# jiamiya/HOPE

Hardware: AMD Instinct MI355X
Metric: parallel env steps/sec (full CarParking step incl. obs + RS search) (higher is better)
Workload: dtype f64

## Files before the change

hope_amd/_lib.py:

```python
import ctypes as C
import os

from .build import lib_path

LIDAR_NUM, N_ACTION, N_ITER, UPSAMPLE, TARGET_DIM, RS_MAX_SEG = 120, 42, 10, 10, 5, 5
F_OBS_F64, F_ACTION_F64, F_PROFILE, F_IMAGE, F_OVERLAP = 0x1, 0x2, 0x4, 0x8, 0x10
STAGE_MOTION, STAGE_OBS, STAGE_REWARD, STAGE_RS, STAGE_ALL = 0x1, 0x2, 0x4, 0x8, 0xF
ACTION_PHYSICAL = 0x10
ACTION_RESCALE_F32 = 0x80
AUTO_REDRAW = 0x100
DEFER_RS = 0x200
STAGE_IMG = 0x40
STAGE_NO_CULL, STAGE_ONE_SCENE = 0x4000, 0x8000
IMG_SIZE, IMG_CHANNELS, TRAJ_RENDER_LEN = 64, 3, 20
AUTO_RESET = 0x20
KERNELS = ('k_kinematics', 'k_env_step', 'k_rs_words', 'k_rs_validate', 'k_bev_image', 'k_bev_prep', 'k_rs_compact', 'k_post', 'k_rs_segs', 'k_rs_screen')
ABI_VERSION = 8

EXPORTS = ['hope_env_create', 'hope_env_destroy', 'hope_last_error', 'hope_abi_version', 'hope_env_upload_tables',
           'hope_env_set_scenes', 'hope_env_step', 'hope_env_wait_rs', 'hope_env_last_step', 'hope_env_wait_rs_step', 'hope_env_download_n_obst', 'hope_env_queue_check', 'hope_env_reset_obs', 'hope_env_download_state',
           'hope_env_upload_state', 'hope_env_restart', 'hope_env_set_pool', 'hope_env_pool_staging', 'hope_env_commit_pool', 'hope_env_commit_pool_relaxed', 'hope_env_pool_staging_ready', 'hope_env_pool_generation', 'hope_env_redraw', 'hope_env_set_redraw_seed', 'hope_env_download_pool_index', 'hope_env_set_dlp_cases', 'hope_env_pool_overflow', 'hope_env_set_draw_class', 'hope_env_download_scenes', 'hope_env_download_pool_state', 'hope_env_restore_maps', 'hope_env_kernel_ms', 'hope_env_kernel_union_ms', 'hope_env_profile_kernels', 'hope_debug_math', 'hope_debug_geom', 'hope_debug_traffic', 'hope_debug_mask_lut', 'hope_debug_rs_prof', 'hope_debug_rs_log', 'hope_debug_rs_filter_stats', 'hope_debug_rs_filter_dump', 'hope_debug_step_prof', 'hope_debug_census', 'hope_scenegen_generate', 'hope_scenegen_default_threads', 'hope_scenegen_generate_det', 'hope_scenegen_generate_device', 'hope_scenegen_log_det', 'hope_env_generate_pool', 'hope_env_curriculum_enable', 'hope_env_curriculum_disable', 'hope_env_set_pool_buckets', 'hope_env_curriculum_tally', 'hope_env_curriculum_update', 'hope_env_curriculum_state', 'hope_env_curriculum_set_windows', 'hope_env_curriculum_download_lists', 'hope_curriculum_lists_host', 'hope_curriculum_fold_host', 'hope_map_level_host', 'hope_map_level_device', 'hope_env_map_level', 'hope_env_planner_enable', 'hope_env_planner_disable', 'hope_env_planner_reset', 'hope_env_planner_step', 'hope_planner_step_host', 'hope_env_planner_download_state', 'hope_env_chooser_enable', 'hope_env_chooser_disable', 'hope_env_choose', 'hope_chooser_host', 'hope_env_obsnorm_enable', 'hope_env_obsnorm_disable', 'hope_env_obsnorm_set', 'hope_env_obsnorm_get', 'hope_env_obsnorm', 'hope_obsnorm_host', 'hope_env_num_scenes', 'hope_env_max_obstacles', 'hope_env_device_arch']


CURRICULUM_LIST_LEN = 1 << 20
PLAN_STATE_WORDS, PLAN_STEP_RATIO, PLAN_FORCED, PLAN_NO_POP = 6, 1.25, 0x1, 0x2
CHOOSE_NOMASK, CHOOSE_FIXED, CHOOSE_FALLBACK = 64, 128, 10
OBSNORM_LIDAR, OBSNORM_TARGET, OBSNORM_COLS, OBSNORM_UPDATE, OBSNORM_NORMALIZE = 120, 5, 125, 0x1, 0x2
BUCKET_UNLABELLED = 255


class HopeError(RuntimeError):
    pass


class StepOut(C.Structure):
    _fields_ = [('lidar', C.c_void_p), ('action_mask', C.c_void_p), ('target', C.c_void_p), ('reward', C.c_void_p),
# ... 130 lines not shown
```

hope_amd/csrc/hope_env.hip:

```cpp
#include <hip/hip_runtime.h>
#include <math.h>
#include <stdio.h>
#include <stdlib.h>
#include <string.h>

#include <algorithm>
#include <chrono>
#include <string>
#include <vector>

#include "hope_dev.h"
#include "hope_env.h"
#include "hope_internal.h"
#include "hope_step_kernel.h"
#include "hope_obs_pair.h"
#include "hope_motion_pair.h"
#include "hope_scenegen_kernel.h"
#include "hope_curriculum_kernel.h"
#include "hope_maplevel_kernel.h"
#include "hope_planner_kernel.h"
#include "hope_chooser_kernel.h"
#include "hope_obsnorm_kernel.h"

using namespace hope;
// ... 860 lines not shown
    hipError_t e = hipDeviceSynchronize();
    if (e == hipSuccess) e = hipMemcpyFromSymbol(buf, HIP_SYMBOL(g_census), sizeof(buf));
    for (int i = 0; i < 16; i++) {
        const bool is_min = i == 1 || i == 3 || i == 7;
        out[i] = is_min ? ~0ull : 0;
        for (int sh = 0; sh < 64; sh++) out[i] = is_min ? std::min<uint64_t>(out[i], buf[sh * 16 + i]) : out[i] + buf[sh * 16 + i];
    }
    if (e == hipSuccess && reset) {
        for (int sh = 0; sh < 64; sh++) for (int i = 0; i < 16; i++) buf[sh * 16 + i] = (i == 1 || i == 3 || i == 7) ? 0x7ff0000000000000ull : 0;
        e = hipMemcpyToSymbol(HIP_SYMBOL(g_census), buf, sizeof(buf));
    }
    return e == hipSuccess ? HOPE_OK : fail(HOPE_EHIP, std::string("hope_debug_census: ") + hipGetErrorString(e));
}

int hope_debug_rs_prof(uint64_t* out, int reset) {
    hipError_t e = rs_prof_read((unsigned long long*)out, reset);
    return e == hipSuccess ? HOPE_OK : fail(HOPE_EHIP, std::string("hope_debug_rs_prof: ") + hipGetErrorString(e));
}

int hope_debug_rs_filter_stats(uint64_t* out, int reset) {
    if (!out) return fail(HOPE_EINVAL, "hope_debug_rs_filter_stats: null argument");
    hipError_t e = rs_fstat_read((unsigned long long*)out, reset);
    return e == hipSuccess ? HOPE_OK : fail(HOPE_EHIP, std::string("hope_debug_rs_filter_stats: ") + hipGetErrorString(e));
}

int hope_debug_rs_filter_dump(double* out) {
    if (!out) return fail(HOPE_EINVAL, "hope_debug_rs_filter_dump: null argument");
    hipError_t e = rs_fdump_read(out);
    return e == hipSuccess ? HOPE_OK : fail(HOPE_EHIP, std::string("hope_debug_rs_filter_dump: ") + hipGetErrorString(e));
}

int hope_debug_rs_log(int32_t* out, int cap, int32_t* n, int reset) {
// ... 1914 lines not shown
```

hope_amd/csrc/hope_internal.h:

```cpp
#pragma once
#include <hip/hip_runtime.h>
#include <stdint.h>
#include "hope_env.h"

namespace hope {

constexpr uint32_t STAGE_NO_BEAMS = 0x1000;
constexpr uint32_t STAGE_NO_MASK = 0x2000;
constexpr uint32_t STAGE_NO_CULL = 0x4000;
constexpr uint32_t STAGE_ONE_SCENE = 0x8000;

struct RsWord {
    double len[5];
    double Lm;
    int code;
    int n;
    double pad;
};
constexpr int RS_WORDS_PER_SCENE = 48;
constexpr int RS_LIST_MAX_SCENES = 1 << 24;
__host__ __device__ inline int rs_list_pack(int scene, int n_obst) { return (int)(((unsigned)scene << 8) | (unsigned)n_obst); }
__host__ __device__ inline int rs_list_scene(int entry) { return (int)((unsigned)entry >> 8); }
__host__ __device__ inline int rs_list_n_obst(int entry) { return (int)((unsigned)entry & 0xFFu); }
constexpr int RS_IN_WORDS = 14;
// ... 50 lines not shown
    uint8_t* dyn;
    int32_t* layer_valid;
    int32_t* legacy_list;
    int32_t* rebuild;
    int* scratch;
    const uint8_t* active;
    uint8_t* img;
    int debug;
};

struct LaunchTimer {
    virtual void begin(int kind, hipStream_t s) = 0;
    virtual void end(hipStream_t s) = 0;
};
hipError_t launch_rs_search(const RsParams& p, hipStream_t stream, LaunchTimer* timer);
hipError_t rs_prof_read(unsigned long long* out , int reset);
hipError_t rs_init_tables();
hipError_t rs_fstat_read(unsigned long long* out , int reset);
hipError_t rs_fdump_read(double* out );
hipError_t rs_log_read(int* out , int cap, int* n, int reset);
size_t rs_lds_bytes(int max_obst);
size_t rs_screen_lds_bytes(int max_obst);
size_t rs_rec_bytes_per_scene();
hipError_t launch_bev_image(const BevParams& p, hipStream_t stream, LaunchTimer* timer, hipStream_t side = nullptr, hipEvent_t ev_fork = nullptr,
                            hipEvent_t ev_join = nullptr);
size_t bev_lds_bytes(bool legacy);

}
```

hope_amd/csrc/hope_rs.hip:

```cpp
#include <stdlib.h>

#include "hope_dev.h"
#include "hope_internal.h"

namespace hope {

namespace {

constexpr double MAXC = RS_MAXC;
constexpr double RS_STEP = 0.1;
constexpr double MAX_LENGTH = 1000.0;
constexpr int NCAND = 46;

enum { TS = 0, TL = 1, TR = 2 };

__device__ __forceinline__ double py_mod(double v, double w) {
    double m = hm_fmod(v, w);
    if (m != 0) { if ((w < 0) != (m < 0)) m += w; } else m = copysign(0.0, w);
    return m;
}
__device__ __forceinline__ double rs_M(double theta) {
    double phi = py_mod(theta, 2.0 * PI);
    if (phi < -PI) phi += 2.0 * PI;
    if (phi > PI) phi -= 2.0 * PI;
// ... 175 lines not shown
    v = fmaxf(v, dpp_f<0x141>(v));
    v = fmaxf(v, dpp_f<0x140>(v));
    const int i = __float_as_int(v);
    return fmaxf(fmaxf(__int_as_float(__builtin_amdgcn_readlane(i, 0)), __int_as_float(__builtin_amdgcn_readlane(i, 16))),
                 fmaxf(__int_as_float(__builtin_amdgcn_readlane(i, 32)), __int_as_float(__builtin_amdgcn_readlane(i, 48))));
}

__device__ __forceinline__ double wave_min_d(double v) {
    v = fmin(v, __hiloint2double(__builtin_amdgcn_mov_dpp(__double2hiint(v), 0xB1, 0xf, 0xf, true), __builtin_amdgcn_mov_dpp(__double2loint(v), 0xB1, 0xf, 0xf, true)));
    v = fmin(v, __hiloint2double(__builtin_amdgcn_mov_dpp(__double2hiint(v), 0x4E, 0xf, 0xf, true), __builtin_amdgcn_mov_dpp(__double2loint(v), 0x4E, 0xf, 0xf, true)));
    v = fmin(v, __hiloint2double(__builtin_amdgcn_mov_dpp(__double2hiint(v), 0x141, 0xf, 0xf, true), __builtin_amdgcn_mov_dpp(__double2loint(v), 0x141, 0xf, 0xf, true)));
    v = fmin(v, __hiloint2double(__builtin_amdgcn_mov_dpp(__double2hiint(v), 0x140, 0xf, 0xf, true), __builtin_amdgcn_mov_dpp(__double2loint(v), 0x140, 0xf, 0xf, true)));
    return fmin(fmin(readlane_d(v, 0), readlane_d(v, 16)), fmin(readlane_d(v, 32), readlane_d(v, 48)));
}

__device__ unsigned long long g_rs_prof[64 * 16];
constexpr int RS_LOG_CAP = 1 << 21;
__device__ int g_rs_log_n;
__device__ int4 g_rs_log[RS_LOG_CAP];
#define RS_T0() unsigned long long t0_ = TIMING ? __builtin_readcyclecounter() : 0
#define RS_T(i) do { if (TIMING) { const unsigned long long t1_ = __builtin_readcyclecounter(); tsec[i] += t1_ - t0_; t0_ = t1_; } } while (0)

template <bool TIMING, bool FULL = false>
__device__ __forceinline__ bool pose_hits(bool active, double wx, double wy, double wyaw, const double* tile,
                                          const float4* obb, int* cand, int n_obst, double xmin, double xmax,
                                          double ymin, double ymax, int lane, unsigned long long* tsec) {
    RS_T0();
    bool bad = false;
    double vx[4], vy[4];
    double hminx = INFINITY, hmaxx = -INFINITY, hminy = INFINITY, hmaxy = -INFINITY;
    if (active) {
// ... 322 lines not shown
        }
        if (k == 0) {
            tb[RS_SEGW + 7] = cq0;
            tb[2 * RS_SEGW + 7] = -sq0;
        }
    }
}

constexpr int RSB_SEG = 0, RSB_SEGW = RS_SEGW, RSB_QPD = RS_SEG_TABLE, RSB_QCAP = 256, RSB_BAD = RSB_QPD + RSB_QCAP;
constexpr int RSB_WORDS = RSB_BAD + 8;

template <int OCC, bool TIMING>
__global__ __launch_bounds__(64, OCC) void k_rs_validate(RsParams p, int obs_f64) {
    extern __shared__ __attribute__((aligned(16))) double lds[];
    const int lane = threadIdx.x;
    unsigned long long tsec[16] = {};
    const unsigned long long tstart_ = TIMING ? __builtin_readcyclecounter() : 0;
    RS_T0();
    const int count = *p.rs_count;
    if ((int)blockIdx.x >= count) return;
    if (obs_f64 & 0x400) return;
    const int qidx = scene_of_block(blockIdx.x, count);
    const int slot = p.slot_base + p.slot_dir * qidx;
    double* tile = lds;
    float4* obb = (float4*)(lds + 8 * p.tile_cap);
    double* scr = lds + 10 * p.tile_cap;
    double* segp = scr + RSB_SEG;
    double* qpd = scr + RSB_QPD;
    int* cand = (int*)(scr + RSB_WORDS);
    unsigned char* qseg = (unsigned char*)(cand + ((p.tile_cap + 3) & ~3));

// ... 125 lines not shown
                double cd = 0;
                unsigned char cs = 0;
                if (lane < rem) { cd = qpd[n + lane]; cs = qseg[n + lane]; }
                wsync();
                if (lane < rem) { qpd[lane] = cd; qseg[lane] = cs; }
                nq = rem;
            }
            wsync();
        }
        if (!invalid) { found = idx - 1; break; }
    }
    if (TIMING) {
        tsec[6] = __builtin_readcyclecounter() - tstart_;
        tsec[8] = 1;
        if (lane == 0) {
            for (int i = 0; i < 16; i++) if (tsec[i]) atomicAdd(&g_rs_prof[(blockIdx.x & 63) * 16 + i], tsec[i]);
            const int li = atomicAdd(&g_rs_log_n, 1);
            if (li < RS_LOG_CAP) g_rs_log[li] = make_int4((int)tsec[6], (int)tsec[9] | (n_paths << 8) | ((p.tile_cap > 32) << 16), (int)tsec[11], found >= 0);
        }
    }
    if (found < 0) return;

    const double wlen = lane < 5 ? segp[RSB_SEGW * lane + 6] : 0.0;
    const int code = __double2loint(segp[7]), nseg = __double2hiint(segp[7]);
    if (lane < 5) {
        double lm = lane < nseg ? wlen / MAXC : 0.0;
        if (p.rs_lengths) {
            if (obs_f64 & 1) ((double*)p.rs_lengths)[5 * (size_t)scene + lane] = lm;
            else ((float*)p.rs_lengths)[5 * (size_t)scene + lane] = (float)lm;
        }
        p.rs_word[8 * (size_t)scene + lane] = lane < nseg ? (int8_t)type_of(code, lane) : (int8_t)HOPE_RS_NONE;
    }
    if (lane == 5) p.rs_word[8 * (size_t)scene + 5] = (int8_t)nseg;
    if (lane == 6) p.rs_word[8 * (size_t)scene + 6] = 1;
}


constexpr float FEPS = 1e-3f, FKAPPA = 2e-2f, FETA_HULL = 2e-3f;
constexpr float F_INV_MAXC = (float)(1.0 / MAXC);
constexpr float F_HL = (float)(0.5 * (CAR_XF - CAR_XR)), F_HW = (float)CAR_YH, F_MID = (float)(0.5 * (CAR_XF + CAR_XR));
constexpr int RS_TAB = 256;
constexpr int RSB_TABF = RSB_BAD + 8, RSB_WORDS_F = RSB_TABF + RS_TAB;
constexpr int RSF_OCC = 4;
__device__ double g_rs_steps[RS_TAB];
__device__ unsigned long long g_rs_fstat[16];
__device__ double g_rs_fdump[64 * 16];

template <bool FULL>
__device__ __noinline__ bool exact_pass(int idx, const double* segp, const double* qpd, const unsigned char* qseg, double c_q,
                                        double s_q, double q0x, double q0y, double q0w, const double* verts_g,
                                        const float4* obb_g, int* cand, int n_obst, double xmin, double xmax, double ymin,
                                        double ymax, int lane) {
    const bool active = idx >= 0;
    double px = 0, py = 0, pyaw = 0;
    if (active) {
        const double spd = qpd[idx];
        const double* sp_ = segp + RSB_SEGW * (int)qseg[idx];
        const int m = (int)sp_[5];
        interpolate(spd, m, sp_[0], sp_[1], sp_[2], sp_[3], -sp_[4], sp_[3], sp_[4], px, py, pyaw);
// ... 67 lines not shown
            }
        }
    }
    return bad;
}

__device__ __forceinline__ double uni_d(double v) {
    return __hiloint2double(__builtin_amdgcn_readfirstlane(__double2hiint(v)), __builtin_amdgcn_readfirstlane(__double2loint(v)));
}

__device__ __forceinline__ void lsync() {
    asm volatile("s_waitcnt lgkmcnt(0)" ::: "memory");
    __builtin_amdgcn_wave_barrier();
}

constexpr double SCREEN_EPS = 1e-7;
constexpr int SCREEN_SPAN = 128;

__device__ __forceinline__ bool screen_obstacle_hit(const float4 v01, const float4 v23, float cx, float cy, float hc, float hs,
                                                    int efl, bool hull_ok) {
    constexpr float FEPS_ = FEPS, FKAPPA_ = FKAPPA, HL = F_HL, HW = F_HW;
    float u[4], w[4];
    {
        const float dx0 = v01.x - cx, dy0 = v01.y - cy, dx1 = v01.z - cx, dy1 = v01.w - cy;
        const float dx2 = v23.x - cx, dy2 = v23.y - cy, dx3 = v23.z - cx, dy3 = v23.w - cy;
        u[0] = hc * dx0 + hs * dy0; w[0] = hc * dy0 - hs * dx0;
        u[1] = hc * dx1 + hs * dy1; w[1] = hc * dy1 - hs * dx1;
        u[2] = hc * dx2 + hs * dy2; w[2] = hc * dy2 - hs * dx2;
        u[3] = hc * dx3 + hs * dy3; w[3] = hc * dy3 - hs * dx3;
    }
// ... 14 lines not shown
        const float ew0 = fminf(w[k], w[k2]), ew1 = fmaxf(w[k], w[k2]);
        const float esep = fmaxf(fmaxf(eu0 - HL, -HL - eu1), fmaxf(ew0 - HW, -HW - ew1));
        const float n1 = fabsf(nu) + fabsf(nw), mg = FEPS_ * n1;
        const bool clear = dn > mg || esep > FEPS_ || fmaxf(g[k], g[k2]) < -FEPS_;
        const bool cross = dn < -mg && esep < -FEPS_ && fminf(fabsf(g[k]), fabsf(g[k2])) > FEPS_ && fmaxf(g[k], g[k2]) > FEPS_;
        const float A = fabsf(nu) * HL, B = fabsf(nw) * HW;
        const bool corners_ok = fminf(fabsf(dn), fabsf(dist - fabsf(A - B))) > mg;
        const bool cross_u = fabsf(dist - A) <= B + mg, cross_w = fabsf(dist - B) <= A + mg;
        const bool angle_ok = (!cross_u || fabsf(nw) >= FKAPPA_ * n1) && (!cross_w || fabsf(nu) >= FKAPPA_ * n1);
        hit = hit || (!clear && cross && corners_ok && angle_ok && hull_ok && ((efl >> k) & 1));
    }
    return hit;
}

template <bool TIMING>
__device__ __forceinline__ unsigned long long screen_words(int lane, int n_paths, int n_obst, const double* tables, double* qpd, int* pq, int* cand,
                                                           const float2* fv, const float4* fbox, const unsigned char* eflag, float fxmax,
                                                           float fymax, unsigned long long* tsec) {
    const float fxmin = 0.0f, fymin = 0.0f;
    const double step = RS_STEP * MAXC;
    unsigned long long condemned = 0;
    RS_T0();
    const double inv_step = 1.0 / step;
    for (int w0 = 0; w0 < n_paths; w0 += 4) {
        const int nw = min(4, n_paths - w0);
        if (w0 > 0)
            for (int t = lane; t < RS_SEG_TABLE * nw; t += WAVE) qpd[t] = tables[RS_SEG_TABLE * w0 + t];
        lsync();
        RS_T(14);
        const int G = nw == 1 ? 64 : (nw == 2 ? 32 : (nw == 3 ? 21 : 16));
        const int stride = SCREEN_SPAN / G;
        const int wl_ = nw == 1 ? 0 : (nw == 2 ? lane >> 5 : (nw == 3 ? (lane >= 42 ? 2 : (lane >= 21 ? 1 : 0)) : lane >> 4));
        const int kk = lane - wl_ * G;
        const double* T = qpd + RS_SEG_TABLE * wl_;
        const double w7s = T[7];
        const int codew = __double2loint(w7s), nsegw = __double2hiint(w7s);
        const double a = (double)((kk + 1) * stride) * step;
        double c = 0.0, u0 = step, r = 0.0, lprev = 0.0, pdv = 0.0;
        int si = -1;
#pragma unroll
        for (int i = 0; i < 5; i++) {
            if (i < nsegw) {
                const double l = T[RS_SEGW * i + 6], al = fabs(l);
                if (i >= 1) u0 = (lprev * l > 0) ? r : -r;
// ... 78 lines not shown
                    classify(WAVE);
                    if (dead == all_w) { npq = 0; break; }
                    const int rem = npq - WAVE;
                    int cv = 0;
                    if (lane < rem) cv = pq[WAVE + lane];
                    lsync();
                    if (lane < rem) pq[lane] = cv;
                    npq = rem;
                }
            }
            if (npq > 0 && dead != all_w) { lsync(); classify(npq); }
        }
        condemned |= (unsigned long long)dead << w0;
        lsync();
        RS_T(7);
    }
    return condemned;
}

template <bool TIMING, int OCC = 8>
__global__ __launch_bounds__(64, OCC) void k_rs_screen(RsParams p) {
    extern __shared__ __attribute__((aligned(16))) double lds[];
    const int lane = threadIdx.x;
    unsigned long long tsec[16] = {};
    const int b_ = (int)blockIdx.x;
    const int qidx = scene_of_block(b_, p.max_queue);
    const int entry = p.rs_list[qidx];
    const int count = *p.rs_count;
    if (qidx >= count) return;
    const int slot = p.slot_base + p.slot_dir * qidx;
    const int scene = rs_list_scene(entry), n_obst = rs_list_n_obst(entry);
    float2* fv = (float2*)lds;
    float4* fbox = (float4*)(lds + 4 * p.tile_cap);
    double* tabs = lds + 6 * p.tile_cap;
    int* pq = (int*)(tabs + 4 * RS_SEG_TABLE);
    int* cand = pq + 2 * WAVE;
    unsigned char* eflag = (unsigned char*)(cand + ((p.tile_cap + 3) & ~3));
    double* rec = p.rs_rec + (size_t)slot * RS_REC_DOUBLES;
    const double r0 = lane < RS_REC_HDR ? rec[lane] : 0.0;
    const double* tables = rec + RS_REC_SEGS;
    {
        typedef __attribute__((address_space(3))) void* lds_ptr;
        const double2* t2 = (const double2*)tables;
        __builtin_amdgcn_global_load_lds((const void*)(t2 + lane), (lds_ptr)tabs, 16, 0, 0);
        if (lane < 2 * RS_SEG_TABLE - WAVE) __builtin_amdgcn_global_load_lds((const void*)(t2 + WAVE + lane), (lds_ptr)(tabs + 2 * WAVE), 16, 0, 0);
        const float4* gfv = p.fverts + (size_t)scene * p.max_obst * 2;
        const float4* gfb = p.fbox + (size_t)scene * p.max_obst;
        const uint32_t* gfl = (const uint32_t*)(p.eflag + (size_t)scene * eflag_stride(p.max_obst));
        float4* lfv = (float4*)fv;
        for (int base = 0; base < 2 * n_obst; base += WAVE)
            if (base + lane < 2 * n_obst) __builtin_amdgcn_global_load_lds((const void*)(gfv + base + lane), (lds_ptr)(lfv + base), 16, 0, 0);
        for (int base = 0; base < n_obst; base += WAVE)
            if (base + lane < n_obst) __builtin_amdgcn_global_load_lds((const void*)(gfb + base + lane), (lds_ptr)(fbox + base), 16, 0, 0);
        for (int base = 0; 4 * base < n_obst; base += WAVE)
            if (4 * (base + lane) < n_obst) __builtin_amdgcn_global_load_lds((const void*)(gfl + base + lane), (lds_ptr)((uint32_t*)eflag + base), 4, 0, 0);
    }
    asm volatile("s_waitcnt vmcnt(0)" ::: "memory");
    const int n_paths = __builtin_amdgcn_readlane(__double2hiint(r0), 1);
    if (n_paths == 0) return;
    const float fxmax = (float)(readlane_d(r0, 6) - readlane_d(r0, 5)), fymax = (float)(readlane_d(r0, 8) - readlane_d(r0, 7));
    lsync();
    const unsigned long long condemned = screen_words<TIMING>(lane, n_paths, n_obst, tables, tabs, pq, cand, fv, fbox, eflag, fxmax, fymax, tsec);
    if (lane == 0) {
        ((unsigned long long*)rec)[9] = condemned;
        if (condemned != ((1ull << n_paths) - 1)) p.surv_list[atomicAdd(p.surv_count, 1)] = make_int2(qidx, entry);
    }
}

template <int OCC, bool TIMING, bool STATS, bool PRE = false>
__global__ __launch_bounds__(64, OCC) void k_rs_validate_f(RsParams p, int obs_f64) {
    extern __shared__ __attribute__((aligned(16))) double lds[];
    const int lane = threadIdx.x;
    if (!(obs_f64 & 0x10000)) __builtin_amdgcn_s_setprio(1);
    unsigned long long tsec[16] = {};
    const unsigned long long tstart_ = TIMING ? __builtin_readcyclecounter() : 0;
    RS_T0();
    const int b_ = (int)blockIdx.x;
    int qidx, entry;
    if (PRE) {
        const int2 sv = p.surv_list[b_];
        if (b_ >= *p.surv_count) return;
        qidx = sv.x; entry = sv.y;
    } else {
#ifdef HOPE_RS_3TRIPS
        const int count = *p.rs_count;
        if (b_ >= count) return;
        qidx = scene_of_block(b_, count);
        entry = p.rs_list[qidx];
#else
// ... 17 lines not shown
    double* tabl = scr + RSB_TABF;
    unsigned char* qseg = (unsigned char*)(cand + ((p.tile_cap + 3) & ~3));
    unsigned char* eflag = qseg + RSB_QCAP;

    const double* rec = p.rs_rec + (size_t)slot * RS_REC_DOUBLES;
    const double r0 = lane < RS_REC_HDR ? rec[lane] : 0.0;
    const double* tables = rec + RS_REC_SEGS;
#ifdef HOPE_RS_3TRIPS
    if (__builtin_amdgcn_readlane(__double2hiint(r0), 1) == 0) return;
#endif
#ifdef HOPE_RS_HDR
    const int scene = __builtin_amdgcn_readlane(__double2loint(r0), 0);
    const int n_obst = __builtin_amdgcn_readlane(__double2hiint(r0), 0);
    (void)entry;
#endif
    double tb = lane < RS_SEG_TABLE ? tables[lane] : 0.0;
    if (!PRE) {
        typedef __attribute__((address_space(3))) void* lds_ptr;
        const double2* t2 = (const double2*)tables;
        __builtin_amdgcn_global_load_lds((const void*)(t2 + lane), (lds_ptr)qpd, 16, 0, 0);
        if (lane < 2 * RS_SEG_TABLE - WAVE) __builtin_amdgcn_global_load_lds((const void*)(t2 + WAVE + lane), (lds_ptr)(qpd + 2 * WAVE), 16, 0, 0);
    }
    {
        typedef __attribute__((address_space(3))) void* lds_ptr;
        const float4* gfv = p.fverts + (size_t)scene * p.max_obst * 2;
        const float4* gfb = p.fbox + (size_t)scene * p.max_obst;
        const uint32_t* gfl = (const uint32_t*)(p.eflag + (size_t)scene * eflag_stride(p.max_obst));
        float4* lfv = (float4*)fv;
        for (int base = 0; base < 2 * n_obst; base += WAVE)
            if (base + lane < 2 * n_obst) __builtin_amdgcn_global_load_lds((const void*)(gfv + base + lane), (lds_ptr)(lfv + base), 16, 0, 0);
        for (int base = 0; base < n_obst; base += WAVE)
            if (base + lane < n_obst) __builtin_amdgcn_global_load_lds((const void*)(gfb + base + lane), (lds_ptr)(fbox + base), 16, 0, 0);
        for (int base = 0; 4 * base < n_obst; base += WAVE)
            if (4 * (base + lane) < n_obst) __builtin_amdgcn_global_load_lds((const void*)(gfl + base + lane), (lds_ptr)((uint32_t*)eflag + base), 4, 0, 0);
    }
    const int n_paths = __builtin_amdgcn_readlane(__double2hiint(r0), 1);
    if (n_paths == 0) {
        asm volatile("s_waitcnt vmcnt(0)" ::: "memory");
        return;
    }
    const double* verts_g = p.verts + (size_t)scene * p.max_obst * 8;
    const float fxmin = 0.0f, fxmax = (float)(readlane_d(r0, 6) - readlane_d(r0, 5)), fymin = 0.0f, fymax = (float)(readlane_d(r0, 8) - readlane_d(r0, 7));
    const double step = RS_STEP * MAXC;
    bool tile_pending = true;
    int found = -1;
    double* bad1 = scr + RSB_BAD;
    if (lane < 6) bad1[lane] = INFINITY;
    lsync();
    RS_T(0);
    const bool paranoid = (obs_f64 & 0x2000) != 0;
    unsigned long long st_pass = 0, st_hit = 0, st_exact = 0, st_unc = 0, st_bad_hit = 0, st_bad_clear = 0, st_samples = 0;
    unsigned long long st_why[5] = {};
    unsigned long long condemned = 0;
    if (PRE) condemned = (unsigned long long)__double_as_longlong(readlane_d(r0, 9));
    else if (!(obs_f64 & 0x20000)) {
        asm volatile("s_waitcnt vmcnt(0)" ::: "memory");
        tile_pending = false;
        condemned = screen_words<TIMING>(lane, n_paths, n_obst, tables, qpd, (int*)tabl ,
                                         cand, fv, fbox, eflag, fxmax, fymax, tsec);
        if (TIMING) t0_ = __builtin_readcyclecounter();
    }
    else {
        asm volatile("s_waitcnt vmcnt(0)" ::: "memory");
        tile_pending = false;
    }
    const bool verify_screen = STATS && paranoid;
    const bool all_condemned = condemned == ((1ull << n_paths) - 1);
    unsigned long long st_scr_words = __popcll(condemned), st_scr_dead = all_condemned ? 1 : 0, st_scr_bad = 0;
    if (!all_condemned || verify_screen) {
        const double T0 = g_rs_steps[lane], T1 = g_rs_steps[WAVE + lane], T2 = g_rs_steps[2 * WAVE + lane], T3 = g_rs_steps[3 * WAVE + lane];
        tabl[lane] = T0; tabl[WAVE + lane] = T1; tabl[2 * WAVE + lane] = T2; tabl[3 * WAVE + lane] = T3;
        lsync();
    }
    for (int idx = 1; idx <= n_paths; idx++) {
        if (all_condemned && !verify_screen) break;
        const double tcur = tb;
        if (idx < n_paths && lane < RS_SEG_TABLE) tb = tables[RS_SEG_TABLE * idx + lane];
        const double len0 = readlane_d(tcur, 6), w6 = readlane_d(tcur, 7);
        const int code = __double2loint(w6), nseg = __double2hiint(w6);
        const int cls1 = type_of(code, 0) * 2 + (len0 > 0.0 ? 1 : 0);
        if (fabs(len0) >= bad1[cls1]) continue;
        const bool screened = (condemned >> (idx - 1)) & 1;
        if (screened && !verify_screen) continue;
        bool invalid = false;
        if (lane < RS_SEG_TABLE) segp[lane] = tcur;
        if (TIMING) tsec[9] += 1;
        {
            double zero;
            asm volatile("v_mov_b64 %0, 0" : "=v"(zero));
            if (lane == 0) { qpd[0] = zero; qseg[0] = (unsigned char)__double2loint(zero); }
        }
        int nq = 1;
        lsync();
        RS_T(1);
        const int win = 128;
        int i = 0, t_off = 0;
        bool seg_open = false, finished = false;
        double pd = 0, ll = 0.0, lprev = 0.0, d = 0, l = 0;
        while (!invalid && (!finished || nq > 0)) {
            while (!finished && nq + WAVE + 1 <= win) {
                if (TIMING) tsec[10] += 1;
                if (!seg_open) {
                    l = uni_d(segp[RSB_SEGW * i + 6]);
                    d = uni_d(l > 0.0 ? step : -step);
                    pd = uni_d((i >= 1 && (lprev * l) > 0) ? -d - ll : d - ll);
                    lprev = l;
                    seg_open = true;
                }
                double mine, t = pd;
                int ncap;
                if (i == 0 && t_off + WAVE <= RS_TAB) {
                    const double v = tabl[t_off + lane];
                    mine = d > 0.0 ? v : -v;
                    ncap = WAVE;
                    t_off += WAVE;
                    if (t_off < RS_TAB) {
                        const double nx = tabl[t_off];
                        t = d > 0.0 ? nx : -nx;
                    } else t = readlane_d(mine, WAVE - 1) + d;
                } else {
                    mine = pd;
                    double last = pd;
                    ncap = 0;
                    for (int j0 = 0; j0 < WAVE; j0 += 8) {
                        if ((lane >> 3) == (j0 >> 3)) mine = t;
#pragma unroll
                        for (int jj = 0; jj < 7; jj++) t = t + d;
                        last = t;
                        t = t + d;
                        ncap = j0 + 8;
                        if (__any(fabs(last) > fabs(l))) break;
                    }
#pragma unroll
                    for (int k = 0; k < 7; k++)
                        if (k < (lane & 7)) mine = mine + d;
                }
                const bool in_seg = lane < ncap && fabs(mine) <= fabs(l);
                const unsigned long long valid = (ncap == WAVE) ? ~0ull : ((1ull << ncap) - 1);
                const unsigned long long fail = ~__ballot(in_seg) & valid;
                const int cnt = fail ? (__ffsll((long long)fail) - 1) : ncap;
                if (lane < cnt) { qpd[nq + lane] = mine; qseg[nq + lane] = (unsigned char)i; }
                nq += cnt;
                if (fail) {
                    pd = readlane_d(mine, cnt);
                    ll = uni_d(l - pd - d);
                    seg_open = false;
                    if (i == nseg - 1) {
                        if (lane == 0) { qpd[nq] = l; qseg[nq] = (unsigned char)i; }
                        nq += 1;
                        finished = true;
// ... 184 lines not shown
            }
            {
                const int rem = n_all - n;
                double cd = 0;
                unsigned char cs = 0;
                if (lane < rem) { cd = qpd[n + lane]; cs = qseg[n + lane]; }
                lsync();
                if (lane < rem) { qpd[lane] = cd; qseg[lane] = cs; }
                nq = rem;
            }
            lsync();
        }
        if (STATS && screened && !invalid) { st_scr_bad += 1; continue; }
        if (!invalid) { found = idx - 1; break; }
    }
    if (STATS && lane == 0) {
        atomicAdd(&g_rs_fstat[7], st_scr_bad); atomicAdd(&g_rs_fstat[13], st_scr_words); atomicAdd(&g_rs_fstat[14], st_scr_dead);
        for (int b = 0; b < 5; b++) atomicAdd(&g_rs_fstat[8 + b], st_why[b]);
        atomicAdd(&g_rs_fstat[0], st_pass); atomicAdd(&g_rs_fstat[1], st_hit); atomicAdd(&g_rs_fstat[2], st_exact);
        atomicAdd(&g_rs_fstat[3], st_unc); atomicAdd(&g_rs_fstat[4], st_bad_hit); atomicAdd(&g_rs_fstat[5], st_bad_clear);
        atomicAdd(&g_rs_fstat[6], st_samples);
    }
    if (TIMING) {
        tsec[6] = __builtin_readcyclecounter() - tstart_;
        tsec[8] = 1;
        if (lane == 0) {
            for (int i = 0; i < 16; i++) if (tsec[i]) atomicAdd(&g_rs_prof[(blockIdx.x & 63) * 16 + i], tsec[i]);
            const int li = atomicAdd(&g_rs_log_n, 1);
            if (li < RS_LOG_CAP) g_rs_log[li] = make_int4((int)tsec[6], (int)tsec[9] | (n_paths << 8) | ((p.tile_cap > 32) << 16), (int)tsec[11], found >= 0);
        }
    }
    if (found < 0) return;
    const double wlen = lane < 5 ? segp[RSB_SEGW * lane + 6] : 0.0;
    const int code = __double2loint(segp[7]), nseg = __double2hiint(segp[7]);
    if (lane < 5) {
        double lm = lane < nseg ? wlen / MAXC : 0.0;
        if (p.rs_lengths) {
            if (obs_f64 & 1) ((double*)p.rs_lengths)[5 * (size_t)scene + lane] = lm;
            else ((float*)p.rs_lengths)[5 * (size_t)scene + lane] = (float)lm;
        }
        p.rs_word[8 * (size_t)scene + lane] = lane < nseg ? (int8_t)type_of(code, lane) : (int8_t)HOPE_RS_NONE;
    }
    if (lane == 5) p.rs_word[8 * (size_t)scene + 5] = (int8_t)nseg;
    if (lane == 6) p.rs_word[8 * (size_t)scene + 6] = 1;
}

}

static size_t rs_lds_bytes_exact(int max_obst) {
    return (size_t)(10 * max_obst + RSB_WORDS) * 8 + (size_t)((max_obst + 3) & ~3) * 4 + RSB_QCAP;
}
static size_t rs_lds_bytes_filter(int max_obst) {
    return (size_t)(6 * max_obst + RSB_WORDS_F) * 8 + (size_t)((max_obst + 3) & ~3) * 4 + RSB_QCAP + (size_t)((max_obst + 3) & ~3);
}
size_t rs_lds_bytes(int max_obst) { return std::max(rs_lds_bytes_exact(max_obst), rs_lds_bytes_filter(max_obst)); }
size_t rs_screen_lds_bytes(int max_obst) {
    return (size_t)(6 * max_obst + 4 * RS_SEG_TABLE) * 8 + 2 * WAVE * 4 + (size_t)((max_obst + 3) & ~3) * 4 + (size_t)((max_obst + 3) & ~3);
}
size_t rs_rec_bytes_per_scene() { return sizeof(double) * RS_REC_DOUBLES; }

hipError_t rs_prof_read(unsigned long long* out, int reset) {
    hipError_t e = hipDeviceSynchronize();
    if (e != hipSuccess) return e;
    static unsigned long long buf[64 * 16];
    e = hipMemcpyFromSymbol(buf, HIP_SYMBOL(g_rs_prof), sizeof(buf));
    for (int i = 0; i < 16; i++) { out[i] = 0; for (int sh = 0; sh < 64; sh++) out[i] += buf[sh * 16 + i]; }
    if (e == hipSuccess && reset) {
        for (auto& v : buf) v = 0;
        e = hipMemcpyToSymbol(HIP_SYMBOL(g_rs_prof), buf, sizeof(buf));
    }
    return e;
}

hipError_t rs_fdump_read(double* out ) {
    hipError_t e = hipDeviceSynchronize();
    if (e != hipSuccess) return e;
    return hipMemcpyFromSymbol(out, HIP_SYMBOL(g_rs_fdump), sizeof(double) * 64 * 16);
}

hipError_t rs_log_read(int* out , int cap, int* n, int reset) {
    hipError_t e = hipDeviceSynchronize();
// ... 87 lines not shown
```

include/hope_env.h:

```cpp
#ifndef HOPE_ENV_H
#define HOPE_ENV_H

#include <stdint.h>

#ifdef __cplusplus
extern "C" {
#endif

#define HOPE_ABI_VERSION 8

#define HOPE_LIDAR_NUM 120
#define HOPE_N_ACTION 42
#define HOPE_N_ITER 10
#define HOPE_UPSAMPLE 10
#define HOPE_TARGET_DIM 5
#define HOPE_RS_MAX_SEG 5
#define HOPE_IMG_SIZE 64
#define HOPE_IMG_CHANNELS 3
#define HOPE_TRAJ_RENDER_LEN 20

#define HOPE_OK 0
#define HOPE_EINVAL (-1)
#define HOPE_ENODEV (-2)
#define HOPE_ENOMEM (-3)
// ... 111 lines not shown
int hope_env_profile_kernels(hope_env_t *h, uint32_t kernel_mask);

int hope_env_download_state(hope_env_t *h, double *pose , int32_t *t ,
                            double *accum );
int hope_env_upload_state(hope_env_t *h, const double *pose, const int32_t *t, const double *accum);

int hope_debug_math(int fn, int n, const double *a, const double *b, double *out, void *stream);

int hope_debug_geom(int fn, int n, int n_obst, const double *in, void *out, void *stream);

int hope_debug_mask_lut(const double *dist_star, const double *hull_base, uint16_t *lut_out, double *scale_out);

int hope_debug_traffic(int mode, size_t bytes, void *buf, void *stream);

int hope_debug_rs_prof(uint64_t *out , int reset);
int hope_debug_rs_filter_stats(uint64_t *out , int reset);
int hope_debug_rs_filter_dump(double *out );
int hope_debug_rs_log(int32_t *out , int cap, int32_t *n, int reset);
int hope_debug_step_prof(uint64_t *out , int reset);
int hope_debug_census(uint64_t *out , int reset);

int hope_scenegen_generate(int level, int bay_mode, int n, uint64_t seed, int64_t first_index, int max_obstacles, double *start,
                           double *dest, double *bbox, double *verts, int32_t *n_obst, int32_t *case_id, int n_threads);
int hope_scenegen_default_threads(void);

int hope_scenegen_generate_det(int level, int bay_mode, int n, uint64_t seed, int64_t first_index, int max_obstacles, double *start,
                               double *dest, double *bbox, double *verts, int32_t *n_obst, int32_t *case_id, int n_threads);
int hope_scenegen_generate_device(int device_id, int level, int bay_mode, int n, uint64_t seed, int64_t first_index, int max_obstacles,
                                  double *start, double *dest, double *bbox, double *verts, int32_t *n_obst, int32_t *case_id, void *stream);
int hope_scenegen_log_det(int n, const double *x, double *y);
// ... 88 lines not shown
```

Measured before the change: 151.5 million.

## Double-buffer RS screen tables via LDS DMA and walk only surviving words

The screen loop now prefetches the next group of four word tables into a second LDS buffer with global_load_lds_dwordx4 while the current group is screened, instead of copying them with plain loads after a sync. The validate walk iterates only over uncondemned words using a bitmask, prefetching the next surviving word's table and reusing the table still resident in LDS. The step-sample table is loaded lazily by async DMA only when a word is actually walked, so fully condemned scenes skip it. It also adds more profiling slots and a walk-profile debug export. In exchange the screen kernel uses more LDS, which may lower occupancy, and the inline asm adds synchronisation subtleties.

```diff
diff --git a/hope_amd/_lib.py b/hope_amd/_lib.py
--- a/hope_amd/_lib.py
+++ b/hope_amd/_lib.py
@@ -19,7 +19,7 @@
 
 EXPORTS = ['hope_env_create', 'hope_env_destroy', 'hope_last_error', 'hope_abi_version', 'hope_env_upload_tables',
            'hope_env_set_scenes', 'hope_env_step', 'hope_env_wait_rs', 'hope_env_last_step', 'hope_env_wait_rs_step', 'hope_env_download_n_obst', 'hope_env_queue_check', 'hope_env_reset_obs', 'hope_env_download_state',
-           'hope_env_upload_state', 'hope_env_restart', 'hope_env_set_pool', 'hope_env_pool_staging', 'hope_env_commit_pool', 'hope_env_commit_pool_relaxed', 'hope_env_pool_staging_ready', 'hope_env_pool_generation', 'hope_env_redraw', 'hope_env_set_redraw_seed', 'hope_env_download_pool_index', 'hope_env_set_dlp_cases', 'hope_env_pool_overflow', 'hope_env_set_draw_class', 'hope_env_download_scenes', 'hope_env_download_pool_state', 'hope_env_restore_maps', 'hope_env_kernel_ms', 'hope_env_kernel_union_ms', 'hope_env_profile_kernels', 'hope_debug_math', 'hope_debug_geom', 'hope_debug_traffic', 'hope_debug_mask_lut', 'hope_debug_rs_prof', 'hope_debug_rs_log', 'hope_debug_rs_filter_stats', 'hope_debug_rs_filter_dump', 'hope_debug_step_prof', 'hope_debug_census', 'hope_scenegen_generate', 'hope_scenegen_default_threads', 'hope_scenegen_generate_det', 'hope_scenegen_generate_device', 'hope_scenegen_log_det', 'hope_env_generate_pool', 'hope_env_curriculum_enable', 'hope_env_curriculum_disable', 'hope_env_set_pool_buckets', 'hope_env_curriculum_tally', 'hope_env_curriculum_update', 'hope_env_curriculum_state', 'hope_env_curriculum_set_windows', 'hope_env_curriculum_download_lists', 'hope_curriculum_lists_host', 'hope_curriculum_fold_host', 'hope_map_level_host', 'hope_map_level_device', 'hope_env_map_level', 'hope_env_planner_enable', 'hope_env_planner_disable', 'hope_env_planner_reset', 'hope_env_planner_step', 'hope_planner_step_host', 'hope_env_planner_download_state', 'hope_env_chooser_enable', 'hope_env_chooser_disable', 'hope_env_choose', 'hope_chooser_host', 'hope_env_obsnorm_enable', 'hope_env_obsnorm_disable', 'hope_env_obsnorm_set', 'hope_env_obsnorm_get', 'hope_env_obsnorm', 'hope_obsnorm_host', 'hope_env_num_scenes', 'hope_env_max_obstacles', 'hope_env_device_arch']
+           'hope_env_upload_state', 'hope_env_restart', 'hope_env_set_pool', 'hope_env_pool_staging', 'hope_env_commit_pool', 'hope_env_commit_pool_relaxed', 'hope_env_pool_staging_ready', 'hope_env_pool_generation', 'hope_env_redraw', 'hope_env_set_redraw_seed', 'hope_env_download_pool_index', 'hope_env_set_dlp_cases', 'hope_env_pool_overflow', 'hope_env_set_draw_class', 'hope_env_download_scenes', 'hope_env_download_pool_state', 'hope_env_restore_maps', 'hope_env_kernel_ms', 'hope_env_kernel_union_ms', 'hope_env_profile_kernels', 'hope_debug_math', 'hope_debug_geom', 'hope_debug_traffic', 'hope_debug_mask_lut', 'hope_debug_rs_prof', 'hope_debug_rs_walk_prof', 'hope_debug_rs_log', 'hope_debug_rs_filter_stats', 'hope_debug_rs_filter_dump', 'hope_debug_step_prof', 'hope_debug_census', 'hope_scenegen_generate', 'hope_scenegen_default_threads', 'hope_scenegen_generate_det', 'hope_scenegen_generate_device', 'hope_scenegen_log_det', 'hope_env_generate_pool', 'hope_env_curriculum_enable', 'hope_env_curriculum_disable', 'hope_env_set_pool_buckets', 'hope_env_curriculum_tally', 'hope_env_curriculum_update', 'hope_env_curriculum_state', 'hope_env_curriculum_set_windows', 'hope_env_curriculum_download_lists', 'hope_curriculum_lists_host', 'hope_curriculum_fold_host', 'hope_map_level_host', 'hope_map_level_device', 'hope_env_map_level', 'hope_env_planner_enable', 'hope_env_planner_disable', 'hope_env_planner_reset', 'hope_env_planner_step', 'hope_planner_step_host', 'hope_env_planner_download_state', 'hope_env_chooser_enable', 'hope_env_chooser_disable', 'hope_env_choose', 'hope_chooser_host', 'hope_env_obsnorm_enable', 'hope_env_obsnorm_disable', 'hope_env_obsnorm_set', 'hope_env_obsnorm_get', 'hope_env_obsnorm', 'hope_obsnorm_host', 'hope_env_num_scenes', 'hope_env_max_obstacles', 'hope_env_device_arch']
 
 
 CURRICULUM_LIST_LEN = 1 << 20
diff --git a/hope_amd/csrc/hope_env.hip b/hope_amd/csrc/hope_env.hip
--- a/hope_amd/csrc/hope_env.hip
+++ b/hope_amd/csrc/hope_env.hip
@@ -898,8 +898,13 @@
 }
 
 int hope_debug_rs_prof(uint64_t* out, int reset) {
-    hipError_t e = rs_prof_read((unsigned long long*)out, reset);
+    hipError_t e = rs_prof_read((unsigned long long*)out, 0, 16, reset);
     return e == hipSuccess ? HOPE_OK : fail(HOPE_EHIP, std::string("hope_debug_rs_prof: ") + hipGetErrorString(e));
+}
+
+int hope_debug_rs_walk_prof(uint64_t* out, int reset) {
+    hipError_t e = rs_prof_read((unsigned long long*)out, 16, 8, reset);
+    return e == hipSuccess ? HOPE_OK : fail(HOPE_EHIP, std::string("hope_debug_rs_walk_prof: ") + hipGetErrorString(e));
 }
 
 int hope_debug_rs_filter_stats(uint64_t* out, int reset) {
diff --git a/hope_amd/csrc/hope_internal.h b/hope_amd/csrc/hope_internal.h
--- a/hope_amd/csrc/hope_internal.h
+++ b/hope_amd/csrc/hope_internal.h
@@ -88,7 +88,7 @@
     virtual void end(hipStream_t s) = 0;
 };
 hipError_t launch_rs_search(const RsParams& p, hipStream_t stream, LaunchTimer* timer);
-hipError_t rs_prof_read(unsigned long long* out , int reset);
+hipError_t rs_prof_read(unsigned long long* out , int first, int count, int reset);
 hipError_t rs_init_tables();
 hipError_t rs_fstat_read(unsigned long long* out , int reset);
 hipError_t rs_fdump_read(double* out );
diff --git a/hope_amd/csrc/hope_rs.hip b/hope_amd/csrc/hope_rs.hip
--- a/hope_amd/csrc/hope_rs.hip
+++ b/hope_amd/csrc/hope_rs.hip
@@ -213,7 +213,8 @@
     return fmin(fmin(readlane_d(v, 0), readlane_d(v, 16)), fmin(readlane_d(v, 32), readlane_d(v, 48)));
 }
 
-__device__ unsigned long long g_rs_prof[64 * 16];
+constexpr int RS_PROF_SLOTS = 24;
+__device__ unsigned long long g_rs_prof[64 * RS_PROF_SLOTS];
 constexpr int RS_LOG_CAP = 1 << 21;
 __device__ int g_rs_log_n;
 __device__ int4 g_rs_log[RS_LOG_CAP];
@@ -566,7 +567,7 @@
 __global__ __launch_bounds__(64, OCC) void k_rs_validate(RsParams p, int obs_f64) {
     extern __shared__ __attribute__((aligned(16))) double lds[];
     const int lane = threadIdx.x;
-    unsigned long long tsec[16] = {};
+    unsigned long long tsec[RS_PROF_SLOTS] = {};
     const unsigned long long tstart_ = TIMING ? __builtin_readcyclecounter() : 0;
     RS_T0();
     const int count = *p.rs_count;
@@ -722,7 +723,7 @@
         tsec[6] = __builtin_readcyclecounter() - tstart_;
         tsec[8] = 1;
         if (lane == 0) {
-            for (int i = 0; i < 16; i++) if (tsec[i]) atomicAdd(&g_rs_prof[(blockIdx.x & 63) * 16 + i], tsec[i]);
+            for (int i = 0; i < RS_PROF_SLOTS; i++) if (tsec[i]) atomicAdd(&g_rs_prof[(blockIdx.x & 63) * RS_PROF_SLOTS + i], tsec[i]);
             const int li = atomicAdd(&g_rs_log_n, 1);
             if (li < RS_LOG_CAP) g_rs_log[li] = make_int4((int)tsec[6], (int)tsec[9] | (n_paths << 8) | ((p.tile_cap > 32) << 16), (int)tsec[11], found >= 0);
         }
@@ -749,8 +750,10 @@
 constexpr float F_HL = (float)(0.5 * (CAR_XF - CAR_XR)), F_HW = (float)CAR_YH, F_MID = (float)(0.5 * (CAR_XF + CAR_XR));
 constexpr int RS_TAB = 256;
 constexpr int RSB_TABF = RSB_BAD + 8, RSB_WORDS_F = RSB_TABF + RS_TAB;
+constexpr int RSB_TABS2 = RSB_QPD + 4 * RS_SEG_TABLE, RSB_PQ = RSB_TABS2 + 4 * RS_SEG_TABLE;
+static_assert(RSB_PQ + WAVE <= RSB_TABF + RS_TAB, "the screen's second table buffer and pair queue (128 ints) end inside the sample table's words");
 constexpr int RSF_OCC = 4;
-__device__ double g_rs_steps[RS_TAB];
+__device__ __attribute__((aligned(16))) double g_rs_steps[RS_TAB];
 __device__ unsigned long long g_rs_fstat[16];
 __device__ double g_rs_fdump[64 * 16];
 
@@ -848,6 +851,19 @@
     __builtin_amdgcn_wave_barrier();
 }
 
+#pragma clang diagnostic push
+#pragma clang diagnostic ignored "-Winline-asm"
+__device__ __forceinline__ void lds_dma16(const void* src, const void* dst, int lane) {
+    typedef __attribute__((address_space(3))) const void* lds_cptr;
+    const unsigned m = __builtin_amdgcn_readfirstlane((unsigned)(unsigned long)(lds_cptr)dst);
+    const unsigned long a = (unsigned long)src;
+    const unsigned long sa = ((unsigned long)(unsigned)__builtin_amdgcn_readfirstlane((int)(a >> 32)) << 32) | (unsigned)__builtin_amdgcn_readfirstlane((int)a);
+    unsigned off;
+    asm volatile("s_mov_b32 m0, %2\n\tv_lshlrev_b32 %0, 4, %1\n\tglobal_load_lds_dwordx4 %0, %3"
+                 : "=&v"(off) : "v"(lane), "s"(m), "s"(sa) : "memory", "m0");
+}
+#pragma clang diagnostic pop
+
 constexpr double SCREEN_EPS = 1e-7;
 constexpr int SCREEN_SPAN = 128;
 
@@ -892,9 +908,9 @@
 }
 
 template <bool TIMING>
-__device__ __forceinline__ unsigned long long screen_words(int lane, int n_paths, int n_obst, const double* tables, double* qpd, int* pq, int* cand,
-                                                           const float2* fv, const float4* fbox, const unsigned char* eflag, float fxmax,
-                                                           float fymax, unsigned long long* tsec) {
+__device__ __forceinline__ unsigned long long screen_words(int lane, int n_paths, int n_obst, const double* tables, double* qpd, double* qpd2,
+                                                           int* pq, int* cand, const float2* fv, const float4* fbox, const unsigned char* eflag,
+                                                           float fxmax, float fymax, unsigned long long* tsec, const double** resident) {
     const float fxmin = 0.0f, fymin = 0.0f;
     const double step = RS_STEP * MAXC;
     unsigned long long condemned = 0;
@@ -902,10 +918,16 @@
     const double inv_step = 1.0 / step;
     for (int w0 = 0; w0 < n_paths; w0 += 4) {
         const int nw = min(4, n_paths - w0);
-        if (w0 > 0)
-            for (int t = lane; t < RS_SEG_TABLE * nw; t += WAVE) qpd[t] = tables[RS_SEG_TABLE * w0 + t];
+        if (w0 > 0) asm volatile("s_waitcnt vmcnt(0)" ::: "memory");
         lsync();
+        if (TIMING && w0 > 0) { tsec[19] += __builtin_readcyclecounter() - t0_; tsec[22] += 1; }
         RS_T(14);
+        if (w0 + 4 < n_paths) {
+            const int n2 = (RS_SEG_TABLE / 2) * min(4, n_paths - w0 - 4);
+            const double2* t2 = (const double2*)(tables + RS_SEG_TABLE * (w0 + 4));
+            if (lane < n2) lds_dma16(t2, qpd2, lane);
+            if (WAVE + lane < n2) lds_dma16(t2 + WAVE, qpd2 + 2 * WAVE, lane);
+        }
         const int G = nw == 1 ? 64 : (nw == 2 ? 32 : (nw == 3 ? 21 : 16));
         const int stride = SCREEN_SPAN / G;
         const int wl_ = nw == 1 ? 0 : (nw == 2 ? lane >> 5 : (nw == 3 ? (lane >= 42 ? 2 : (lane >= 21 ? 1 : 0)) : lane >> 4));
@@ -1014,7 +1036,9 @@
         condemned |= (unsigned long long)dead << w0;
         lsync();
         RS_T(7);
-    }
+        if (w0 + 4 < n_paths) { double* sw = qpd; qpd = qpd2; qpd2 = sw; }
+    }
+    *resident = qpd;
     return condemned;
 }
 
@@ -1022,7 +1046,7 @@
 __global__ __launch_bounds__(64, OCC) void k_rs_screen(RsParams p) {
     extern __shared__ __attribute__((aligned(16))) double lds[];
     const int lane = threadIdx.x;
-    unsigned long long tsec[16] = {};
+    unsigned long long tsec[RS_PROF_SLOTS] = {};
     const int b_ = (int)blockIdx.x;
     const int qidx = scene_of_block(b_, p.max_queue);
     const int entry = p.rs_list[qidx];
@@ -1033,7 +1057,7 @@
     float2* fv = (float2*)lds;
     float4* fbox = (float4*)(lds + 4 * p.tile_cap);
     double* tabs = lds + 6 * p.tile_cap;
-    int* pq = (int*)(tabs + 4 * RS_SEG_TABLE);
+    int* pq = (int*)(tabs + 8 * RS_SEG_TABLE);
     int* cand = pq + 2 * WAVE;
     unsigned char* eflag = (unsigned char*)(cand + ((p.tile_cap + 3) & ~3));
     double* rec = p.rs_rec + (size_t)slot * RS_REC_DOUBLES;
@@ -1060,7 +1084,9 @@
     if (n_paths == 0) return;
     const float fxmax = (float)(readlane_d(r0, 6) - readlane_d(r0, 5)), fymax = (float)(readlane_d(r0, 8) - readlane_d(r0, 7));
     lsync();
-    const unsigned long long condemned = screen_words<TIMING>(lane, n_paths, n_obst, tables, tabs, pq, cand, fv, fbox, eflag, fxmax, fymax, tsec);
+    const double* resident;
+    const unsigned long long condemned = screen_words<TIMING>(lane, n_paths, n_obst, tables, tabs, tabs + 4 * RS_SEG_TABLE, pq, cand, fv, fbox, eflag,
+                                                              fxmax, fymax, tsec, &resident);
     if (lane == 0) {
         ((unsigned long long*)rec)[9] = condemned;
         if (condemned != ((1ull << n_paths) - 1)) p.surv_list[atomicAdd(p.surv_count, 1)] = make_int2(qidx, entry);
@@ -1072,7 +1098,7 @@
     extern __shared__ __attribute__((aligned(16))) double lds[];
     const int lane = threadIdx.x;
     if (!(obs_f64 & 0x10000)) __builtin_amdgcn_s_setprio(1);
-    unsigned long long tsec[16] = {};
+    unsigned long long tsec[RS_PROF_SLOTS] = {};
     const unsigned long long tstart_ = TIMING ? __builtin_readcyclecounter() : 0;
     RS_T0();
     const int b_ = (int)blockIdx.x;
@@ -1120,7 +1146,6 @@
     const int n_obst = __builtin_amdgcn_readlane(__double2hiint(r0), 0);
     (void)entry;
 #endif
-    double tb = lane < RS_SEG_TABLE ? tables[lane] : 0.0;
     if (!PRE) {
         typedef __attribute__((address_space(3))) void* lds_ptr;
         const double2* t2 = (const double2*)tables;
@@ -1151,19 +1176,18 @@
     bool tile_pending = true;
     int found = -1;
     double* bad1 = scr + RSB_BAD;
-    if (lane < 6) bad1[lane] = INFINITY;
-    lsync();
     RS_T(0);
     const bool paranoid = (obs_f64 & 0x2000) != 0;
     unsigned long long st_pass = 0, st_hit = 0, st_exact = 0, st_unc = 0, st_bad_hit = 0, st_bad_clear = 0, st_samples = 0;
     unsigned long long st_why[5] = {};
     unsigned long long condemned = 0;
+    const double* resident = qpd;
     if (PRE) condemned = (unsigned long long)__double_as_longlong(readlane_d(r0, 9));
     else if (!(obs_f64 & 0x20000)) {
         asm volatile("s_waitcnt vmcnt(0)" ::: "memory");
         tile_pending = false;
-        condemned = screen_words<TIMING>(lane, n_paths, n_obst, tables, qpd, (int*)tabl ,
-                                         cand, fv, fbox, eflag, fxmax, fymax, tsec);
+        condemned = screen_words<TIMING>(lane, n_paths, n_obst, tables, qpd, scr + RSB_TABS2, (int*)(scr + RSB_PQ) ,
+                                         cand, fv, fbox, eflag, fxmax, fymax, tsec, &resident);
         if (TIMING) t0_ = __builtin_readcyclecounter();
     }
     else {
@@ -1171,23 +1195,50 @@
         tile_pending = false;
     }
     const bool verify_screen = STATS && paranoid;
-    const bool all_condemned = condemned == ((1ull << n_paths) - 1);
+    const unsigned long long all_words = (1ull << n_paths) - 1;
+    const bool all_condemned = condemned == all_words;
     unsigned long long st_scr_words = __popcll(condemned), st_scr_dead = all_condemned ? 1 : 0, st_scr_bad = 0;
-    if (!all_condemned || verify_screen) {
-        const double T0 = g_rs_steps[lane], T1 = g_rs_steps[WAVE + lane], T2 = g_rs_steps[2 * WAVE + lane], T3 = g_rs_steps[3 * WAVE + lane];
-        tabl[lane] = T0; tabl[WAVE + lane] = T1; tabl[2 * WAVE + lane] = T2; tabl[3 * WAVE + lane] = T3;
-        lsync();
-    }
-    for (int idx = 1; idx <= n_paths; idx++) {
-        if (all_condemned && !verify_screen) break;
+    unsigned long long todo = verify_screen ? all_words : (all_words & ~condemned);
+    if (TIMING && todo) tsec[21] += 1;
+    bool tabl_pending = false;
+    double tb = 0.0;
+    if (todo) {
+        const int first = __ffsll((long long)todo) - 1;
+        const int lds_w0 = (PRE || (obs_f64 & 0x20000)) ? 0 : ((n_paths - 1) & ~3);
+        if (!PRE && first >= lds_w0 && first < lds_w0 + 4) {
+            if (lane < RS_SEG_TABLE) tb = resident[RS_SEG_TABLE * (first - lds_w0) + lane];
+        } else if (lane < RS_SEG_TABLE) tb = tables[RS_SEG_TABLE * first + lane];
+    }
+    if (lane < 6) bad1[lane] = INFINITY;
+    lsync();
+    bool walked = false, tabl_requested = false;
+    while (todo) {
+        const unsigned long long tw_ = TIMING ? __builtin_readcyclecounter() : 0;
+        const int idx = __ffsll((long long)todo);
+        todo &= todo - 1;
+        if (tabl_pending && walked) {
+            asm volatile("s_waitcnt vmcnt(0)" ::: "memory");
+            tabl_pending = false;
+        }
         const double tcur = tb;
-        if (idx < n_paths && lane < RS_SEG_TABLE) tb = tables[RS_SEG_TABLE * idx + lane];
+        if (todo && lane < RS_SEG_TABLE) tb = tables[RS_SEG_TABLE * (__ffsll((long long)todo) - 1) + lane];
         const double len0 = readlane_d(tcur, 6), w6 = readlane_d(tcur, 7);
         const int code = __double2loint(w6), nseg = __double2hiint(w6);
+        if (TIMING) asm volatile("" :: "s"(code));
         const int cls1 = type_of(code, 0) * 2 + (len0 > 0.0 ? 1 : 0);
-        if (fabs(len0) >= bad1[cls1]) continue;
+        if (fabs(len0) >= bad1[cls1]) {
+            if (TIMING) { tsec[16] += __builtin_readcyclecounter() - tw_; tsec[20] += 1; }
+            continue;
+        }
         const bool screened = (condemned >> (idx - 1)) & 1;
-        if (screened && !verify_screen) continue;
+        if (!tabl_requested) {
+            const double2* g2 = (const double2*)g_rs_steps;
+            lds_dma16(g2, tabl, lane);
+            lds_dma16(g2 + WAVE, tabl + 2 * WAVE, lane);
+            tabl_requested = tabl_pending = true;
+        }
+        if (TIMING) tsec[18] += __builtin_readcyclecounter() - tw_;
+        walked = true;
         bool invalid = false;
         if (lane < RS_SEG_TABLE) segp[lane] = tcur;
         if (TIMING) tsec[9] += 1;
@@ -1215,7 +1266,17 @@
                 }
                 double mine, t = pd;
                 int ncap;
+#ifdef HOPE_RS_TABLE_WAIT
                 if (i == 0 && t_off + WAVE <= RS_TAB) {
+#else
+                if (i == 0 && t_off + WAVE <= RS_TAB && !(tabl_pending && t_off == 0)) {
+#endif
+                    if (tabl_pending) {
+                        const unsigned long long ts_ = TIMING ? __builtin_readcyclecounter() : 0;
+                        asm volatile("s_waitcnt vmcnt(0)" ::: "memory");
+                        tabl_pending = false;
+                        if (TIMING) tsec[17] += __builtin_readcyclecounter() - ts_;
+                    }
                     const double v = tabl[t_off + lane];
                     mine = d > 0.0 ? v : -v;
                     ncap = WAVE;
@@ -1240,6 +1301,7 @@
 #pragma unroll
                     for (int k = 0; k < 7; k++)
                         if (k < (lane & 7)) mine = mine + d;
+                    if (i == 0) t_off += WAVE;
                 }
                 const bool in_seg = lane < ncap && fabs(mine) <= fabs(l);
                 const unsigned long long valid = (ncap == WAVE) ? ~0ull : ((1ull << ncap) - 1);
@@ -1454,6 +1516,7 @@
         if (STATS && screened && !invalid) { st_scr_bad += 1; continue; }
         if (!invalid) { found = idx - 1; break; }
     }
+    if (tabl_pending) asm volatile("s_waitcnt vmcnt(0)" ::: "memory");
     if (STATS && lane == 0) {
         atomicAdd(&g_rs_fstat[7], st_scr_bad); atomicAdd(&g_rs_fstat[13], st_scr_words); atomicAdd(&g_rs_fstat[14], st_scr_dead);
         for (int b = 0; b < 5; b++) atomicAdd(&g_rs_fstat[8 + b], st_why[b]);
@@ -1465,7 +1528,7 @@
         tsec[6] = __builtin_readcyclecounter() - tstart_;
         tsec[8] = 1;
         if (lane == 0) {
-            for (int i = 0; i < 16; i++) if (tsec[i]) atomicAdd(&g_rs_prof[(blockIdx.x & 63) * 16 + i], tsec[i]);
+            for (int i = 0; i < RS_PROF_SLOTS; i++) if (tsec[i]) atomicAdd(&g_rs_prof[(blockIdx.x & 63) * RS_PROF_SLOTS + i], tsec[i]);
             const int li = atomicAdd(&g_rs_log_n, 1);
             if (li < RS_LOG_CAP) g_rs_log[li] = make_int4((int)tsec[6], (int)tsec[9] | (n_paths << 8) | ((p.tile_cap > 32) << 16), (int)tsec[11], found >= 0);
         }
@@ -1495,16 +1558,17 @@
 }
 size_t rs_lds_bytes(int max_obst) { return std::max(rs_lds_bytes_exact(max_obst), rs_lds_bytes_filter(max_obst)); }
 size_t rs_screen_lds_bytes(int max_obst) {
-    return (size_t)(6 * max_obst + 4 * RS_SEG_TABLE) * 8 + 2 * WAVE * 4 + (size_t)((max_obst + 3) & ~3) * 4 + (size_t)((max_obst + 3) & ~3);
+    return (size_t)(6 * max_obst + 8 * RS_SEG_TABLE) * 8 + 2 * WAVE * 4 + (size_t)((max_obst + 3) & ~3) * 4 + (size_t)((max_obst + 3) & ~3);
 }
 size_t rs_rec_bytes_per_scene() { return sizeof(double) * RS_REC_DOUBLES; }
 
-hipError_t rs_prof_read(unsigned long long* out, int reset) {
+hipError_t rs_prof_read(unsigned long long* out, int first, int count, int reset) {
     hipError_t e = hipDeviceSynchronize();
     if (e != hipSuccess) return e;
-    static unsigned long long buf[64 * 16];
+    if (first < 0 || count < 0 || first + count > RS_PROF_SLOTS) return hipErrorInvalidValue;
+    static unsigned long long buf[64 * RS_PROF_SLOTS];
     e = hipMemcpyFromSymbol(buf, HIP_SYMBOL(g_rs_prof), sizeof(buf));
-    for (int i = 0; i < 16; i++) { out[i] = 0; for (int sh = 0; sh < 64; sh++) out[i] += buf[sh * 16 + i]; }
+    for (int i = 0; i < count; i++) { out[i] = 0; for (int sh = 0; sh < 64; sh++) out[i] += buf[sh * RS_PROF_SLOTS + first + i]; }
     if (e == hipSuccess && reset) {
         for (auto& v : buf) v = 0;
         e = hipMemcpyToSymbol(HIP_SYMBOL(g_rs_prof), buf, sizeof(buf));
diff --git a/include/hope_env.h b/include/hope_env.h
--- a/include/hope_env.h
+++ b/include/hope_env.h
@@ -149,6 +149,7 @@
 int hope_debug_traffic(int mode, size_t bytes, void *buf, void *stream);
 
 int hope_debug_rs_prof(uint64_t *out , int reset);
+int hope_debug_rs_walk_prof(uint64_t *out , int reset);
 int hope_debug_rs_filter_stats(uint64_t *out , int reset);
 int hope_debug_rs_filter_dump(double *out );
 int hope_debug_rs_log(int32_t *out , int cap, int32_t *n, int reset);
```

After: 146.5 million. -3.3%, worse.
